# lukifer23/Matrix0

Hardware: AMD Instinct MI355X
Metric: self-play games/sec at 800 sims/move, ResNet-24 53M; 1/2/4/8 MI355X (higher is better)
Workload: dtype f16

## Files before the change

matrix0_amd/csrc/conv_zs.hip:

```cpp
#include "kernel_common.h"
#include "conv_zs_epilogue.h"
#include "conv_zs_tail.h"

namespace {
constexpr int ZS_A_BYTES = 256 * 128;
constexpr int ZS_WH_BYTES = 320 * 64;
constexpr int ZS_OFF_W = 2 * ZS_A_BYTES;
constexpr int ZS_OFF_Z = ZS_OFF_W + 4 * ZS_WH_BYTES;
constexpr int ZS_OFF_D = ZS_OFF_Z + 8192;
constexpr int ZS_LDS_MAIN = ZS_OFF_D + 4096;
}

#define ZS_FENCE() asm volatile("" ::: "memory")

#ifdef SW_STAMP
__device__ unsigned long long* g_zs_stamp;
#endif

template <ConvEpi EPI, int ACT>
__global__ __launch_bounds__(512) void conv_zs_kernel(GemmArgs a) {
    constexpr int NG = 5, MT = 8;
    extern __shared__ __attribute__((aligned(16))) char smem[];
    char* A_lds = smem;
    char* W_lds = smem + ZS_OFF_W;
    char* Z_lds = smem + ZS_OFF_Z;
    char* D_lds = smem + ZS_OFF_D;

#ifdef SW_STAMP
    const unsigned long long st_entry = __builtin_amdgcn_s_memrealtime();
#endif
    const int tid = threadIdx.x;
    const int lane = tid & 63;
    const int wave = __builtin_amdgcn_readfirstlane(tid >> 6);
    const int wn = wave & 3;
    const int wp = wave >> 2;
    const int m0 = blockIdx.x * 256;
    const int n0 = blockIdx.y * 320;
    const int Cin = a.Cin;
    const int nchunk = Cin >> 6;
    const int NH = nchunk * 18;
    const int c15 = lane & 15;
    const int q = lane >> 4;

    reinterpret_cast<uint4*>(Z_lds)[tid] = make_uint4(0, 0, 0, 0);

    const char* in_bytes = reinterpret_cast<const char*>(a.in);
    const char* w_blk = reinterpret_cast<const char*>(a.w) + (size_t)blockIdx.y * (2 * ZS_WH_BYTES) + lane * 16;
    const size_t w_kt_stride = (size_t)gridDim.y * (2 * ZS_WH_BYTES);

    auto issue_A_piece = [&](int chunk, int qq) __attribute__((always_inline)) {
        const int p = 8 * qq + (lane >> 3);
        const int key = (p & 2) | (((p >> 6) & 1) << 2);
        const char* src = in_bytes + ((size_t)(m0 + p) * Cin + (size_t)chunk * 64) * 2 + 16 * ((lane & 7) ^ key);
        glds16(src, A_lds + (chunk & 1) * ZS_A_BYTES + qq * 1024);
    };
    auto issue_half = [&](int y) __attribute__((always_inline)) {
        const char* src = w_blk + (size_t)(y >> 1) * w_kt_stride + (size_t)(y & 1) * ZS_WH_BYTES;
        char* dst = W_lds + (y & 3) * ZS_WH_BYTES;
        glds16(src + wave * 1024, dst + wave * 1024);
        glds16(src + (8 + wave) * 1024, dst + (8 + wave) * 1024);
        if (wave < 4) glds16(src + (16 + wave) * 1024, dst + (16 + wave) * 1024);
        else glds16(w_blk, D_lds + (wave - 4) * 1024);
    };

    float4v acc[MT][NG];
    static_for<0, MT>([&](auto mi) __attribute__((always_inline)) {
        static_for<0, NG>([&](auto ni) __attribute__((always_inline)) {
            acc[decltype(mi)::value][decltype(ni)::value] = float4v{0.f, 0.f, 0.f, 0.f};
        });
    });

    const int wfx = ((4 - ((c15 >> 2) & 3)) & 3) ^ q;
    const int wrow_off = (wn * 80 + c15) * 64;
    const int lx = c15 & 7;
    const int lb = c15 >> 3;
    const int arow0 = (2 * wp + lb) * 64 + lx;

#pragma unroll
    for (int i = 0; i < 4; ++i) issue_A_piece(0, wave * 4 + i);
    issue_half(0);
    issue_half(1);
    issue_half(2);
    asm volatile("s_waitcnt vmcnt(6) lgkmcnt(0)" ::: "memory");
    __builtin_amdgcn_s_barrier();
    if (wp == 1) __builtin_amdgcn_s_barrier();

    const uint32_t w_lane = (uint32_t)lane * 16u;
    const uint32_t a_lane0 = (uint32_t)(lane >> 3) * (uint32_t)Cin * 2u + 16u * (uint32_t)((lane & 7) ^ ((lane >> 3) & 2));
    const uint32_t a_lane1 = (uint32_t)(lane >> 3) * (uint32_t)Cin * 2u + 16u * (uint32_t)((lane & 7) ^ (((lane >> 3) & 2) | 4));
    const char* w_base = reinterpret_cast<const char*>(a.w) + (size_t)blockIdx.y * (2 * ZS_WH_BYTES) + wave * 1024;
    int t_next = 3;
    const char* w_ptr = w_base + (size_t)1 * w_kt_stride + ZS_WH_BYTES;
    int w_slot = 3 * ZS_WH_BYTES;
    const char* a_ptr = in_bytes;
    int a_dst = 0, a_left = 0;
    auto issue_next = [&](auto G_) __attribute__((always_inline)) {
        constexpr int G = decltype(G_)::value;
        char* dst = W_lds + w_slot + wave * 1024;
        glds16(w_ptr + w_lane, dst);
        glds16(w_ptr + 8192 + w_lane, dst + 8192);
        if constexpr (G == 0) {
            glds16(w_ptr + 16384 + w_lane, dst + 16384);
        } else {
            const bool have = a_left > 0;
            const uint32_t al = ((8 - a_left) & 2) ? a_lane1 : a_lane0;
            glds16((have ? a_ptr : in_bytes) + al, have ? A_lds + a_dst : D_lds + (wave - 4) * 1024);
            a_ptr += have ? (size_t)32 * Cin * 2 : 0;
            a_dst += have ? 4096 : 0;
            a_left -= have ? 1 : 0;
        }
        const bool more = t_next + 1 < NH;
        const size_t inc = (t_next & 1) ? (w_kt_stride - ZS_WH_BYTES) : (size_t)ZS_WH_BYTES;
        w_ptr += more ? inc : 0;
        t_next += 1;
        w_slot = (t_next & 3) * ZS_WH_BYTES;
    };

    int y = 0;
#ifdef SW_STAMP
    const unsigned long long st_c0 = __builtin_amdgcn_s_memtime(), st_r0 = __builtin_amdgcn_s_memrealtime();
#endif
    auto main_loop = [&](auto G_) __attribute__((always_inline)) {
    constexpr int G = decltype(G_)::value;
#pragma unroll 1
    for (int c = 0; c < nchunk; ++c) {
        const char* Ab = A_lds + (c & 1) * ZS_A_BYTES;
        if constexpr (G == 1) {
            a_left = c + 1 < nchunk ? 8 : 0;
            a_ptr = in_bytes + ((size_t)(m0 + 8 * (wave - 4)) * Cin + (size_t)(c + 1) * 64) * 2;
            a_dst = ((c + 1) & 1) * ZS_A_BYTES + (wave - 4) * 1024;
        }
        static_for<0, 3>([&](auto t3_) __attribute__((always_inline)) {
            constexpr int t3 = decltype(t3_)::value;
            constexpr int LO = t3 == 0 ? 1 : 0;
            constexpr int HI = t3 == 2 ? 7 : 8;
            const int rbase = arow0 + (t3 == 2 ? 8 : 0) - 1;
#pragma unroll 1
            for (int dxi = 0; dxi < 3; ++dxi) {
                const int xx = lx + dxi - 1;
                const bool ok = (unsigned)xx < 8u;
                const int key = (xx & 2) | (lb << 2);
                const char* rowp = ok ? Ab + (rbase + dxi) * 128 : Z_lds + (xx & 1) * 128;
                const char* ap0 = rowp + 16 * (key ^ q);
                const char* ap1 = rowp + 16 * (key ^ q ^ 4);
                static_for<0, 2>([&](auto h_) __attribute__((always_inline)) {
                    constexpr int h = decltype(h_)::value;
                    const int yh = y + h;
                    const char* ap = h ? ap1 : ap0;
                    half8 fa[MT], fb[NG];
                    const char* Wb = W_lds + (yh & 3) * ZS_WH_BYTES + wrow_off + 16 * wfx;
                    static_for<LO, HI>([&](auto mi_) __attribute__((always_inline)) {
                        constexpr int mi = decltype(mi_)::value;
                        fa[mi] = *reinterpret_cast<const half8*>(ap + (mi - LO) * 1024);
                    });
                    static_for<0, NG>([&](auto ni_) __attribute__((always_inline)) {
                        constexpr int ni = decltype(ni_)::value;
                        fb[ni] = *reinterpret_cast<const half8*>(Wb + ni * 1024);
                    });
                    ZS_FENCE(); issue_next(G_); ZS_FENCE();
                    asm volatile("s_waitcnt vmcnt(3)" ::: "memory");
                    ZS_FENCE();
                    __builtin_amdgcn_s_barrier();
                    ZS_FENCE();
                    __builtin_amdgcn_s_setprio(1);
                    static_for<0, NG>([&](auto ni_) __attribute__((always_inline)) {
                        constexpr int ni = decltype(ni_)::value;
                        static_for<LO, HI>([&](auto mi_) __attribute__((always_inline)) {
                            constexpr int mi = decltype(mi_)::value;
                            if constexpr (EPI == EPI_TAIL || EPI == EPI_TAIL_PRE)
                                acc[mi][ni] = __builtin_amdgcn_mfma_f32_16x16x32_f16(fa[mi], fb[ni], acc[mi][ni], 0, 0, 0);
                            else
                                acc[mi][ni] = __builtin_amdgcn_mfma_f32_16x16x32_f16(fb[ni], fa[mi], acc[mi][ni], 0, 0, 0);
                        });
                    });
                    __builtin_amdgcn_s_setprio(0);
                    ZS_FENCE();
                    __builtin_amdgcn_s_barrier();
                    ZS_FENCE();
                });
                y += 2;
            }
        });
    }
    };
    if (wp == 0) main_loop(std::integral_constant<int, 0>{});
    else main_loop(std::integral_constant<int, 1>{});
#ifdef SW_STAMP
    if (tid == 0) {
        unsigned long long* o = g_zs_stamp + (size_t)blockIdx.x * 4;
        o[0] = st_c0; o[1] = st_r0; o[2] = __builtin_amdgcn_s_memtime(); o[3] = __builtin_amdgcn_s_memrealtime();
    }
#endif
    asm volatile("s_waitcnt vmcnt(0)" ::: "memory");
    if (wp == 0) __builtin_amdgcn_s_barrier();
    __builtin_amdgcn_s_barrier();

    if constexpr (EPI == EPI_TAIL) zs_tail_epilogue<ACT, false>(acc, a, smem, m0, wp, wn, wave, lane);
    else if constexpr (EPI == EPI_TAIL_PRE) zs_tail_epilogue<ACT, true>(acc, a, smem, m0, wp, wn, wave, lane);
    else zs_tile_epilogue<EPI, ACT>(acc, a, smem + wave * 20480, m0, n0, wp, wn, lane);
#ifdef SW_STAMP
    if (tid == 0) {
        unsigned long long* o = g_zs_stamp + (size_t)gridDim.x * 4 + (size_t)blockIdx.x * 4;
        unsigned hw; asm volatile("s_getreg_b32 %0, hwreg(HW_REG_HW_ID)" : "=s"(hw));
        unsigned xcc; asm volatile("s_getreg_b32 %0, hwreg(HW_REG_XCC_ID)" : "=s"(xcc));
        o[0] = st_entry; o[1] = __builtin_amdgcn_s_memrealtime(); o[2] = hw; o[3] = xcc;
    }
#endif
}

template <ConvEpi EPI, int ACT>
static hipError_t launch_conv_zs_e(const GemmArgs& a, hipStream_t st) {
    const size_t lds = 160 * 1024;
    static DeviceOnce once;
    hipError_t e = once.run([] {
        return hipFuncSetAttribute(reinterpret_cast<const void*>(&conv_zs_kernel<EPI, ACT>),
                                   hipFuncAttributeMaxDynamicSharedMemorySize, 160 * 1024);
    });
    if (e != hipSuccess) return e;
    dim3 grid(a.Mrows / 256, a.Npad / 320);
    hipLaunchKernelGGL((conv_zs_kernel<EPI, ACT>), grid, dim3(512), lds, st, a);
    return hipGetLastError();
}

hipError_t launch_conv_zs(const GemmArgs& a, hipStream_t st) {
    if (a.Cin % 64 != 0 || a.Npad % 320 != 0 || a.Mrows % 256 != 0) return hipErrorInvalidValue;
    if (a.mul != nullptr || a.out_f32 != 0) return hipErrorInvalidValue;
    if ((size_t)a.Mrows * a.ldo * 2 >= ((size_t)1 << 32)) return hipErrorInvalidValue;
    if (a.res != nullptr) {
        if (a.N != 320 || a.Npad != 320 || a.ldo != 320 || a.bias != nullptr || a.out_stats != nullptr) return hipErrorInvalidValue;
        if (a.y2 != nullptr && a.gn_gamma == nullptr) return hipErrorInvalidValue;
        if (a.se_w1 != nullptr && (a.se_wf == nullptr || a.se_hidden < 1 || a.se_hidden > TAIL_SE_HMAX)) return hipErrorInvalidValue;
        if (a.pre_gamma != nullptr) {
            if (a.se_w1 != nullptr) return hipErrorInvalidValue;
            if (a.epi_act == ACT_SILU) return launch_conv_zs_e<EPI_TAIL_PRE, ACT_SILU>(a, st);
            if (a.epi_act == ACT_RELU) return launch_conv_zs_e<EPI_TAIL_PRE, ACT_RELU>(a, st);
            return hipErrorInvalidValue;
        }
        if (a.epi_act == ACT_SILU) return launch_conv_zs_e<EPI_TAIL, ACT_SILU>(a, st);
        if (a.epi_act == ACT_RELU) return launch_conv_zs_e<EPI_TAIL, ACT_RELU>(a, st);
        return hipErrorInvalidValue;
    }
    if (a.gn_gamma != nullptr) {
        if (a.epi_act == ACT_SILU) return launch_conv_zs_e<EPI_GN, ACT_SILU>(a, st);
        if (a.epi_act == ACT_RELU) return launch_conv_zs_e<EPI_GN, ACT_RELU>(a, st);
        return hipErrorInvalidValue;
    }
    return a.epi_act == ACT_NONE ? launch_conv_zs_e<EPI_PLAIN, ACT_NONE>(a, st) : hipErrorInvalidValue;
}
```

Baseline: 1.147.

## Drive conv_zs async load schedule from compile-time table, drop dummy loads

Replaces the runtime-predicated issue_next logic with a constexpr schedule header that decides per tap position how many weight and activation pieces each wave group issues and the exact vmcnt to wait for. Dummy loads into a scratch LDS region, used to keep counts uniform, are removed along with that region, and the last chunk is peeled so no loads are issued past the end. The tap loop is split into specialized bodies where issue patterns differ. This cuts wasted global-to-LDS traffic and per-iteration address arithmetic, at the cost of more code size from specialization.

```diff
diff --git a/matrix0_amd/csrc/conv_zs.hip b/matrix0_amd/csrc/conv_zs.hip
--- a/matrix0_amd/csrc/conv_zs.hip
+++ b/matrix0_amd/csrc/conv_zs.hip
@@ -1,14 +1,16 @@
 #include "kernel_common.h"
 #include "conv_zs_epilogue.h"
 #include "conv_zs_tail.h"
+#include "conv_zs_schedule.h"
 
 namespace {
 constexpr int ZS_A_BYTES = 256 * 128;
 constexpr int ZS_WH_BYTES = 320 * 64;
 constexpr int ZS_OFF_W = 2 * ZS_A_BYTES;
 constexpr int ZS_OFF_Z = ZS_OFF_W + 4 * ZS_WH_BYTES;
-constexpr int ZS_OFF_D = ZS_OFF_Z + 8192;
-constexpr int ZS_LDS_MAIN = ZS_OFF_D + 4096;
+constexpr int ZS_LDS_MAIN = ZS_OFF_Z + 8192;
+static_assert(zs_sched::RING * ZS_WH_BYTES == ZS_OFF_Z - ZS_OFF_W && zs_sched::W_PIECES * 1024 == ZS_WH_BYTES &&
+              zs_sched::A_PIECES * 1024 == ZS_A_BYTES, "conv_zs_schedule.h describes this LDS layout");
 }
 
 #define ZS_FENCE() asm volatile("" ::: "memory")
@@ -24,7 +26,6 @@
     char* A_lds = smem;
     char* W_lds = smem + ZS_OFF_W;
     char* Z_lds = smem + ZS_OFF_Z;
-    char* D_lds = smem + ZS_OFF_D;
 
 #ifdef SW_STAMP
     const unsigned long long st_entry = __builtin_amdgcn_s_memrealtime();
@@ -38,14 +39,12 @@
     const int n0 = blockIdx.y * 320;
     const int Cin = a.Cin;
     const int nchunk = Cin >> 6;
-    const int NH = nchunk * 18;
     const int c15 = lane & 15;
     const int q = lane >> 4;
 
     reinterpret_cast<uint4*>(Z_lds)[tid] = make_uint4(0, 0, 0, 0);
 
     const char* in_bytes = reinterpret_cast<const char*>(a.in);
-    const char* w_blk = reinterpret_cast<const char*>(a.w) + (size_t)blockIdx.y * (2 * ZS_WH_BYTES) + lane * 16;
     const size_t w_kt_stride = (size_t)gridDim.y * (2 * ZS_WH_BYTES);
 
     auto issue_A_piece = [&](int chunk, int qq) __attribute__((always_inline)) {
@@ -54,14 +53,6 @@
         const char* src = in_bytes + ((size_t)(m0 + p) * Cin + (size_t)chunk * 64) * 2 + 16 * ((lane & 7) ^ key);
         glds16(src, A_lds + (chunk & 1) * ZS_A_BYTES + qq * 1024);
     };
-    auto issue_half = [&](int y) __attribute__((always_inline)) {
-        const char* src = w_blk + (size_t)(y >> 1) * w_kt_stride + (size_t)(y & 1) * ZS_WH_BYTES;
-        char* dst = W_lds + (y & 3) * ZS_WH_BYTES;
-        glds16(src + wave * 1024, dst + wave * 1024);
-        glds16(src + (8 + wave) * 1024, dst + (8 + wave) * 1024);
-        if (wave < 4) glds16(src + (16 + wave) * 1024, dst + (16 + wave) * 1024);
-        else glds16(w_blk, D_lds + (wave - 4) * 1024);
-    };
 
     float4v acc[MT][NG];
     static_for<0, MT>([&](auto mi) __attribute__((always_inline)) {
@@ -76,67 +67,58 @@
     const int lb = c15 >> 3;
     const int arow0 = (2 * wp + lb) * 64 + lx;
 
-#pragma unroll
-    for (int i = 0; i < 4; ++i) issue_A_piece(0, wave * 4 + i);
-    issue_half(0);
-    issue_half(1);
-    issue_half(2);
-    asm volatile("s_waitcnt vmcnt(6) lgkmcnt(0)" ::: "memory");
-    __builtin_amdgcn_s_barrier();
-    if (wp == 1) __builtin_amdgcn_s_barrier();
-
     const uint32_t w_lane = (uint32_t)lane * 16u;
     const uint32_t a_lane0 = (uint32_t)(lane >> 3) * (uint32_t)Cin * 2u + 16u * (uint32_t)((lane & 7) ^ ((lane >> 3) & 2));
     const uint32_t a_lane1 = (uint32_t)(lane >> 3) * (uint32_t)Cin * 2u + 16u * (uint32_t)((lane & 7) ^ (((lane >> 3) & 2) | 4));
-    const char* w_base = reinterpret_cast<const char*>(a.w) + (size_t)blockIdx.y * (2 * ZS_WH_BYTES) + wave * 1024;
-    int t_next = 3;
-    const char* w_ptr = w_base + (size_t)1 * w_kt_stride + ZS_WH_BYTES;
-    int w_slot = 3 * ZS_WH_BYTES;
-    const char* a_ptr = in_bytes;
-    int a_dst = 0, a_left = 0;
-    auto issue_next = [&](auto G_) __attribute__((always_inline)) {
-        constexpr int G = decltype(G_)::value;
-        char* dst = W_lds + w_slot + wave * 1024;
-        glds16(w_ptr + w_lane, dst);
-        glds16(w_ptr + 8192 + w_lane, dst + 8192);
-        if constexpr (G == 0) {
-            glds16(w_ptr + 16384 + w_lane, dst + 16384);
-        } else {
-            const bool have = a_left > 0;
-            const uint32_t al = ((8 - a_left) & 2) ? a_lane1 : a_lane0;
-            glds16((have ? a_ptr : in_bytes) + al, have ? A_lds + a_dst : D_lds + (wave - 4) * 1024);
-            a_ptr += have ? (size_t)32 * Cin * 2 : 0;
-            a_dst += have ? 4096 : 0;
-            a_left -= have ? 1 : 0;
-        }
-        const bool more = t_next + 1 < NH;
-        const size_t inc = (t_next & 1) ? (w_kt_stride - ZS_WH_BYTES) : (size_t)ZS_WH_BYTES;
-        w_ptr += more ? inc : 0;
+    const size_t a_band = (size_t)32 * Cin * 2;
+    const char* w_ptr = reinterpret_cast<const char*>(a.w) + (size_t)blockIdx.y * (2 * ZS_WH_BYTES) + wave * 1024;
+    int t_next = 0;
+    const char* a_src = in_bytes;
+    int a_dst = 0;
+
+    int y = 0;
+#ifdef SW_STAMP
+    unsigned long long st_c0 = 0, st_r0 = 0;
+#endif
+    auto run = [&](auto G_) __attribute__((always_inline)) {
+    constexpr int G = decltype(G_)::value;
+    auto issue_w = [&](auto ODD_) __attribute__((always_inline)) {
+        char* dst = W_lds + (t_next & 3) * ZS_WH_BYTES + wave * 1024;
+        static_for<0, zs_sched::zs_w_pieces(G)>([&](auto k_) __attribute__((always_inline)) {
+            constexpr int k = decltype(k_)::value;
+            glds16(w_ptr + k * 8192 + w_lane, dst + k * 8192);
+        });
+        w_ptr += decltype(ODD_)::value ? (w_kt_stride - ZS_WH_BYTES) : (size_t)ZS_WH_BYTES;
         t_next += 1;
-        w_slot = (t_next & 3) * ZS_WH_BYTES;
-    };
-
-    int y = 0;
-#ifdef SW_STAMP
-    const unsigned long long st_c0 = __builtin_amdgcn_s_memtime(), st_r0 = __builtin_amdgcn_s_memrealtime();
-#endif
-    auto main_loop = [&](auto G_) __attribute__((always_inline)) {
-    constexpr int G = decltype(G_)::value;
-#pragma unroll 1
-    for (int c = 0; c < nchunk; ++c) {
-        const char* Ab = A_lds + (c & 1) * ZS_A_BYTES;
-        if constexpr (G == 1) {
-            a_left = c + 1 < nchunk ? 8 : 0;
-            a_ptr = in_bytes + ((size_t)(m0 + 8 * (wave - 4)) * Cin + (size_t)(c + 1) * 64) * 2;
-            a_dst = ((c + 1) & 1) * ZS_A_BYTES + (wave - 4) * 1024;
-        }
-        static_for<0, 3>([&](auto t3_) __attribute__((always_inline)) {
+    };
+
+    static_for<zs_sched::PROLOGUE, 0>([&](auto idx_) __attribute__((always_inline)) {
+        constexpr int idx = decltype(idx_)::value;
+        constexpr zs_sched::ZsIssue is = zs_sched::zs_issue(G, idx, false);
+        static_assert(is.w == zs_sched::zs_w_pieces(G), "every prologue position carries a weight half-tile");
+        static_for<0, is.a>([&](auto i_) __attribute__((always_inline)) {
+            issue_A_piece(0, wave * zs_sched::A_PROLOGUE_PIECES + decltype(i_)::value);
+        });
+        issue_w(std::integral_constant<bool, ((idx - zs_sched::PROLOGUE) & 1) != 0>{});
+    });
+    asm volatile("s_waitcnt vmcnt(%0) lgkmcnt(0)" :: "n"(zs_sched::zs_prologue_wait(G)) : "memory");
+    __builtin_amdgcn_s_barrier();
+    if constexpr (G == 1) __builtin_amdgcn_s_barrier();
+#ifdef SW_STAMP
+    st_c0 = __builtin_amdgcn_s_memtime(); st_r0 = __builtin_amdgcn_s_memrealtime();
+#endif
+
+    auto taps = [&](auto LAST_, auto t3_, auto DLO_, auto DHI_, const char* Ab) __attribute__((always_inline)) {
+            constexpr bool LAST = decltype(LAST_)::value;
+            constexpr int DLO = decltype(DLO_)::value, DHI = decltype(DHI_)::value;
             constexpr int t3 = decltype(t3_)::value;
             constexpr int LO = t3 == 0 ? 1 : 0;
             constexpr int HI = t3 == 2 ? 7 : 8;
             const int rbase = arow0 + (t3 == 2 ? 8 : 0) - 1;
+            int dlo = DLO, dhi = DHI;
+            asm volatile("" : "+s"(dlo), "+s"(dhi));
 #pragma unroll 1
-            for (int dxi = 0; dxi < 3; ++dxi) {
+            for (int dxi = dlo; dxi < dhi; ++dxi) {
                 const int xx = lx + dxi - 1;
                 const bool ok = (unsigned)xx < 8u;
                 const int key = (xx & 2) | (lb << 2);
@@ -145,6 +127,8 @@
                 const char* ap1 = rowp + 16 * (key ^ q ^ 4);
                 static_for<0, 2>([&](auto h_) __attribute__((always_inline)) {
                     constexpr int h = decltype(h_)::value;
+                    constexpr zs_sched::ZsIssue is = zs_sched::zs_issue(G, t3 * 6 + DLO * 2 + h, LAST);
+                    constexpr int in_flight = zs_sched::zs_wait(G, t3 * 6 + DLO * 2 + h, LAST);
                     const int yh = y + h;
                     const char* ap = h ? ap1 : ap0;
                     half8 fa[MT], fb[NG];
@@ -157,8 +141,17 @@
                         constexpr int ni = decltype(ni_)::value;
                         fb[ni] = *reinterpret_cast<const half8*>(Wb + ni * 1024);
                     });
-                    ZS_FENCE(); issue_next(G_); ZS_FENCE();
-                    asm volatile("s_waitcnt vmcnt(3)" ::: "memory");
+                    ZS_FENCE();
+                    if constexpr (is.w != 0) {
+                        static_assert(is.w == zs_sched::zs_w_pieces(G), "a weight half-tile goes out whole or not at all");
+                        issue_w(std::integral_constant<bool, h == 0>{});
+                    }
+                    if constexpr (is.a != 0) {
+                        const int xi = zs_sched::zs_a_piece(t3 * 6 + dxi * 2 + h);
+                        glds16(a_src + (size_t)xi * a_band + (h ? a_lane1 : a_lane0), A_lds + a_dst + xi * 4096);
+                    }
+                    ZS_FENCE();
+                    asm volatile("s_waitcnt vmcnt(%0)" :: "n"(in_flight) : "memory");
                     ZS_FENCE();
                     __builtin_amdgcn_s_barrier();
                     ZS_FENCE();
@@ -180,11 +173,36 @@
                 });
                 y += 2;
             }
-        });
-    }
-    };
-    if (wp == 0) main_loop(std::integral_constant<int, 0>{});
-    else main_loop(std::integral_constant<int, 1>{});
+    };
+    auto chunk = [&](auto LAST_, int c) __attribute__((always_inline)) {
+        constexpr bool LAST = decltype(LAST_)::value;
+        const char* Ab = A_lds + (c & 1) * ZS_A_BYTES;
+        if constexpr (G == 1 && !LAST) {
+            a_src = in_bytes + ((size_t)(m0 + 8 * (wave - 4)) * Cin + (size_t)(c + 1) * 64) * 2;
+            a_dst = ((c + 1) & 1) * ZS_A_BYTES + (wave - 4) * 1024;
+        }
+        static_for<0, 3>([&](auto t3_) __attribute__((always_inline)) {
+            constexpr int t3 = decltype(t3_)::value;
+            constexpr bool s01 = zs_sched::zs_same_body(G, LAST, t3, 0, 1), s12 = zs_sched::zs_same_body(G, LAST, t3, 1, 2);
+            using I0 = std::integral_constant<int, 0>; using I1 = std::integral_constant<int, 1>;
+            using I2 = std::integral_constant<int, 2>; using I3 = std::integral_constant<int, 3>;
+            if constexpr (s01 && s12) {
+                taps(LAST_, t3_, I0{}, I3{}, Ab);
+            } else if constexpr (s01) {
+                taps(LAST_, t3_, I0{}, I2{}, Ab); taps(LAST_, t3_, I2{}, I3{}, Ab);
+            } else if constexpr (s12) {
+                taps(LAST_, t3_, I0{}, I1{}, Ab); taps(LAST_, t3_, I1{}, I3{}, Ab);
+            } else {
+                taps(LAST_, t3_, I0{}, I1{}, Ab); taps(LAST_, t3_, I1{}, I2{}, Ab); taps(LAST_, t3_, I2{}, I3{}, Ab);
+            }
+        });
+    };
+#pragma unroll 1
+    for (int c = 0; c + 1 < nchunk; ++c) chunk(std::false_type{}, c);
+    chunk(std::true_type{}, nchunk - 1);
+    };
+    if (wp == 0) run(std::integral_constant<int, 0>{});
+    else run(std::integral_constant<int, 1>{});
 #ifdef SW_STAMP
     if (tid == 0) {
         unsigned long long* o = g_zs_stamp + (size_t)blockIdx.x * 4;
diff --git a/matrix0_amd/csrc/conv_zs_schedule.h b/matrix0_amd/csrc/conv_zs_schedule.h
--- /dev/null
+++ b/matrix0_amd/csrc/conv_zs_schedule.h
@@ -0,0 +1,62 @@
+#pragma once
+
+namespace zs_sched {
+
+constexpr int HALVES_PER_CHUNK = 18;
+constexpr int AHEAD = 3;
+constexpr int RING = 4;
+constexpr int W_PIECES = 20;
+constexpr int A_PIECES = 32;
+constexpr int A_LOOP_PIECES = 8;
+constexpr int A_PROLOGUE_PIECES = 4;
+constexpr int PROLOGUE = -3;
+
+struct ZsIssue {
+    int w;
+    int a;
+};
+
+constexpr int zs_w_pieces(int group) { return group == 0 ? 3 : 2; }
+
+constexpr ZsIssue zs_issue(int group, int idx, bool last_chunk) {
+    if (idx < 0) return ZsIssue{zs_w_pieces(group), idx == PROLOGUE ? A_PROLOGUE_PIECES : 0};
+    return ZsIssue{last_chunk && idx + AHEAD >= HALVES_PER_CHUNK ? 0 : zs_w_pieces(group),
+                   group == 1 && idx < A_LOOP_PIECES && !last_chunk ? 1 : 0};
+}
+
+constexpr int zs_wait(int group, int idx, bool last_chunk) {
+    return zs_issue(group, idx, last_chunk).w + zs_issue(group, idx, last_chunk).a;
+}
+
+constexpr int zs_prologue_wait(int group) {
+    return zs_wait(group, -2, false) + zs_wait(group, -1, false);
+}
+
+constexpr int zs_a_piece(int idx) {
+    return ((idx >> 1) & 1) + (((idx >> 1) & 2) << 1) + 2 * (idx & 1);
+}
+
+constexpr bool zs_a_pieces_ok() {
+    int seen = 0;
+    for (int idx = 0; idx < A_LOOP_PIECES; ++idx) {
+        const int xi = zs_a_piece(idx);
+        if (xi < 0 || xi >= A_LOOP_PIECES || (xi & 2) != 2 * (idx & 1)) return false;
+        seen |= 1 << xi;
+    }
+    return seen == (1 << A_LOOP_PIECES) - 1;
+}
+static_assert(zs_a_pieces_ok(), "the eight positions carry the eight bands once each, odd boards at odd positions");
+static_assert(4 * A_LOOP_PIECES == A_PIECES && 8 * A_PROLOGUE_PIECES == A_PIECES && 4 * zs_w_pieces(0) + 4 * zs_w_pieces(1) == W_PIECES,
+              "the waves' shares add up to a chunk and to a half-tile");
+
+constexpr int zs_w_piece(int wave, int k) { return 8 * k + wave; }
+
+constexpr bool zs_same_body(int group, bool last_chunk, int t3, int dxa, int dxb) {
+    for (int h = 0; h < 2; ++h) {
+        const ZsIssue x = zs_issue(group, t3 * 6 + dxa * 2 + h, last_chunk), y = zs_issue(group, t3 * 6 + dxb * 2 + h, last_chunk);
+        if (x.w != y.w || x.a != y.a) return false;
+    }
+    return true;
+}
+
+}
```

Result: no change. 1.146 (-0.1%).
